# B-R-P/NMSLIB-ZIG

Hardware: AMD Instinct MI355X
Metric: queries/sec @ recall@10, 1M x 128-D L2, batch=1024; HBM GB/s vs peak (higher is better)
Workload: dtype f16+f32

## Files before the change

nmslib_zig_amd/csrc/engine.cpp:

```cpp
#include "engine.hpp"

#include <algorithm>
#include <chrono>
#include <cmath>
#include <cstring>
#include <fstream>
#include <set>
#include <sstream>
#include <thread>

namespace gfxknn {

using clk = std::chrono::steady_clock;

void hip_check(hipError_t e, const char* what) {
    if (e == hipSuccess) return;
    std::string msg = std::string(what) + ": " + hipGetErrorString(e);
    (void)hipGetLastError();
    throw EngineError(e == hipErrorOutOfMemory ? Err::OutOfMemory : Err::Runtime, msg);
}

ParamSet::ParamSet(const std::vector<std::string>& desc) {
    std::set<std::string> seen;
    for (const std::string& d : desc) {
// ... 142 lines not shown
    if (data_type != 0 && data_type != 2)
        throw EngineError(Err::SpaceIncompatible, "only dense float and dense uint8 data are served by the GPU engine");
    if ((sp == SP_L2SQR_SIFT) != (data_type == 2))
        throw EngineError(Err::SpaceIncompatible, "data type does not match space '" + space + "'");
    thread_pool_size = std::thread::hardware_concurrency();
}

Engine::~Engine() {
    for (auto& pr : prof_events_) {
        (void)hipEventDestroy(pr.first);
        (void)hipEventDestroy(pr.second);
    }
    for (hipEvent_t e : shard_events_) (void)hipEventDestroy(e);
    if (shard_ready_) (void)hipEventDestroy(shard_ready_);
    if (pinned_) (void)hipHostFree(pinned_);
    if (stream_) (void)hipStreamDestroy(stream_);
}

void Engine::prof_begin(hipStream_t s) {
    if (!prof_ || prof_events_.size() >= 65536) return;
    hipEvent_t a, b;
    hip_check(hipEventCreate(&a), "hipEventCreate");
    hip_check(hipEventCreate(&b), "hipEventCreate");
    prof_events_.emplace_back(a, b);
    hip_check(hipEventRecord(a, s), "hipEventRecord");
}
void Engine::prof_end(hipStream_t s) {
    if (!prof_ || prof_events_.empty()) return;
    hip_check(hipEventRecord(prof_events_.back().second, s), "hipEventRecord");
}
void Engine::collect_profile(double* total_ms, uint64_t* launches) {
// ... 871 lines not shown
        if (method_ == Method::Brute) knn_brute(qs, m, k, d_ids + q0 * k, d_dists + q0 * k, cnt, stream);
        else knn_hnsw(qs, m, k, d_ids + q0 * k, d_dists + q0 * k, cnt, stream);
    }
}

void Engine::fast_tile_counts(size_t* tiles, size_t* precise, size_t* fallback) {
    *tiles = *precise = *fallback = 0;
    if (!shards_.empty()) {
        shards_[0]->fast_tile_counts(tiles, precise, fallback);
        return;
    }
    if ((last_path != 1 && last_path != 3) || !fast_flags_ || fast_nqt_ <= 0) return;
    std::vector<int> h((size_t)fast_nqt_ * 2, 0);
    hip_check(hipSetDevice(device_), "hipSetDevice");
    hip_check(hipStreamSynchronize(last_stream_ ? last_stream_ : stream_), "stats");
    hip_check(hipMemcpy(h.data(), fast_flags_, (size_t)fast_nqt_ * (fast_has_precise_ ? 2 : 1) * sizeof(int), hipMemcpyDeviceToHost),
              "stats flags");
    *tiles = (size_t)fast_nqt_;
    for (int i = 0; i < fast_nqt_; ++i) {
        *fallback += h[i] != 0;
        if (fast_has_precise_) *precise += h[(size_t)fast_nqt_ + i] != 0;
    }
}

size_t Engine::hnsw_redone() {
    if (!shards_.empty()) return shards_[0]->hnsw_redone();
    if (last_path != 4 || !hnsw_fix_valid_) return 0;
    int32_t v = 0;
    hip_check(hipSetDevice(device_), "hipSetDevice");
    hip_check(hipStreamSynchronize(last_stream_ ? last_stream_ : stream_), "stats");
// ... 73 lines not shown
                ws_qaux_.ensure((size_t)f.qpad * 16);
                ws_qaug_.ensure((size_t)f.qpad * f.dp * 4);
                hip_check(launch_query_aux_cosc(ws_qpad_.as<float>(), ws_qsel_.as<float>(), f.qpad, ldb, dim_eff, mu_norm_,
                                                ws_qaux_.as<float>(), stream),
                          "query aux");
                hip_check(launch_query_aug_cosc(ws_qsel_.as<float>(), ws_qaux_.as<float>(), (int)nq, f.qpad, ldb, dim_eff,
                                                cosc_lambda_, ws_qaug_.as<float>(), f.dp, stream),
                          "augmented queries");
                qsel = ws_qaug_.as<float>();
            }
            ws_cand_.ensure(bf_cand_elems(f.fallback) * 8);
            ws_cnt_.ensure(bf_cnt_elems(f.fallback) * 4);
            ws_f32_q_.ensure((size_t)f.qpad * f.dp * 2 * 3);
            ws_u8_cand_.ensure(bf_f32_top8_elems(f) * 4);
            ws_u8_thr_.ensure(bf_f32_thr_bytes(f));
            ws_flags_.ensure((size_t)f.fallback.nqt * 4 + 64);
            ws_u8_list_.ensure(bf_f32_list_elems(f) * 4);
            ws_u8_listcnt_.ensure(bf_f32_listcnt_elems(f) * 4);
            float* thr = ws_u8_thr_.as<float>();
            int* tile_fail = reinterpret_cast<int*>(thr + 2 * (size_t)f.qpad);
            char* qh = ws_f32_q_.as<char>();
            char* ql = qh + (size_t)f.qpad * f.dp * 2;
            BfF16Side h16{d_f16_hi_.ptr(), d_auxp16_.as<float>(), ql + (size_t)f.qpad * f.dp * 2, f16_scale_, bres16_, f16_scale_q_};
            hipEvent_t eb = nullptr, ee = nullptr;
            if (prof_ && prof_events_.size() < 65536) {
                hip_check(hipEventCreate(&eb), "hipEventCreate");
                hip_check(hipEventCreate(&ee), "hipEventCreate");
                prof_events_.emplace_back(eb, ee);
            }
            hip_check(launch_bf_f32_fast(f, space_, (int)d_n_, dim_eff, ldb, (int)nq, (int)k, d_rows_.as<float>(),
                                         centred_ ? d_rows_sel_.as<float>() : d_rows_.as<float>(), d_aux_.as<float>(),
                                         d_bf_hi_.ptr(), d_bf_lo_.ptr(), d_auxp_.as<float>(), f.cosc ? bmax_c_ : bmax_,
                                         f.cosc ? bres_c_ : bres_, ws_qpad_.as<float>(), qsel, qh, ql,
                                         ws_u8_cand_.as<float>(), ws_cand_.as<unsigned long long>(), ws_cnt_.as<int>(), thr,
                                         ws_u8_list_.as<uint32_t>(), ws_u8_listcnt_.as<int>(), tile_fail, ws_flags_.as<int>(),
                                         d_ids_.as<int32_t>(), d_ids, d_dists, d_cnt, eb, ee, stream,
                                         centred_ ? nullptr : static_cast<const float*>(d_queries), centred_ ? nullptr : ws_qpad_.as<float>(),
                                         f.cosc ? ws_qaux_.as<float>() : nullptr, f.cosc ? ws_qsel_.as<float>() : nullptr, f.dp, h16),
                      "bf_f32_fast");
            last_path = 1;
            fast_flags_ = tile_fail;
            fast_nqt_ = f.nqt;
            fast_has_precise_ = true;
            return;
        }
    }
    last_path = is_u8() ? 2 : 0;
    BfPlan p = bf_make_plan((int)d_n_, dim_eff, (int)nq, (int)k, is_u8());
    if (d_n_ == 0) p.ldb = is_u8() ? 128 : f32_row_stride(dim_eff);
    const int elem = is_u8() ? 1 : 4;
    ws_qpad_.ensure((size_t)p.qpad * p.ldb * elem);
// ... 180 lines not shown
    return pinned_;
}

Engine::ResultBlock Engine::result_block(size_t nq, size_t k) {
    ws_ids_.ensure(2 * nq * k * 4 + nq * 4);
    int32_t* d_ids = ws_ids_.as<int32_t>();
    return {d_ids, reinterpret_cast<float*>(d_ids + nq * k), d_ids + 2 * nq * k};
}

void Engine::fetch_results(size_t nq, size_t k, const char* what, const int32_t** ids, const float** dists,
                           const int32_t** cnt) {
    const size_t rbytes = nq * k * 4;
    char* hp = static_cast<char*>(pinned_);
    hip_check(hipMemcpyAsync(hp, ws_ids_.ptr(), 2 * rbytes + nq * 4, hipMemcpyDeviceToHost, stream_), "results D2H");
    hip_check(hipStreamSynchronize(stream_), what);
    *ids = reinterpret_cast<const int32_t*>(hp);
    *dists = reinterpret_cast<const float*>(hp + rbytes);
    *cnt = reinterpret_cast<const int32_t*>(hp + 2 * rbytes);
}

void Engine::scan_slices(size_t nq, size_t k, int tq, const ResultBlock& out, const ScanLaunch& launch) {
    const int n = (int)d_n_;
    const size_t max_split_keys = (size_t)1 << 25;
    for (size_t q0 = 0; q0 < nq;) {
        int m = (int)std::min<size_t>(32768, nq - q0);
        ScanPlan p = scan_make_plan(n, m, (int)k, tq);
        while (m > 1 && (size_t)p.nsplit * m * k > max_split_keys) {
            m = std::max(1, m / 2);
            p = scan_make_plan(n, m, (int)k, tq);
        }
// ... 415 lines not shown
```

nmslib_zig_amd/csrc/engine.hpp:

```cpp
#pragma once
#include <hip/hip_runtime_api.h>

#include <cstdint>
#include <functional>
#include <map>
#include <memory>
#include <mutex>
#include <stdexcept>
#include <string>
#include <utility>
#include <vector>

#include "kernels/kernels.hpp"

namespace gfxknn {

enum class Err : int {
    InvalidArgument = 2,
    OutOfMemory = 3,
    SpaceIncompatible = 5,
    QueryTooLarge = 6,
    IndexBuildFailed = 8,
    QueryExecutionFailed = 9,
    DataIO = 10,
// ... 170 lines not shown
    const uint8_t* rows_u8() const { return parent_ ? parent_->rows_u8_.data() + view_lo_ * 128 : rows_u8_.data(); }
    int resolve_shards() const;
    void finalize_sharded(int nshards);
    void knn_sharded(const void* d_queries, size_t nq, size_t elem_count, size_t k, int32_t* d_ids, float* d_dists,
                     int32_t* d_cnt, hipStream_t stream);
    std::vector<std::unique_ptr<Engine>> shards_;
    std::vector<hipEvent_t> shard_events_;
    hipEvent_t shard_ready_ = nullptr;
    const Engine* parent_ = nullptr;
    size_t view_lo_ = 0, view_n_ = 0;
    int forced_device_ = -1;
    int gpu_shards_ = -1;
    DevBuf ws_sh_ids_, ws_sh_d_, ws_bigk_, ws_bigk_tmp_;
    void* pinned(size_t bytes);
    void* pinned_ = nullptr;
    size_t pinned_bytes_ = 0;
    void check_device();
    struct ResultBlock {
        int32_t* ids;
        float* dists;
        int32_t* cnt;
    };
    ResultBlock result_block(size_t nq, size_t k);
    void fetch_results(size_t nq, size_t k, const char* what, const int32_t** ids, const float** dists,
                       const int32_t** cnt);
    using ScanLaunch = std::function<void(const ScanPlan& p, size_t q0, float* split_d, int32_t* split_pos)>;
    void scan_slices(size_t nq, size_t k, int tq, const ResultBlock& out, const ScanLaunch& launch);
    using RangeLaunch = std::function<void(float* filter, float* report)>;
    size_t range_select(bool two_dists, float r, size_t capacity, int32_t* ids, float* dists, const RangeLaunch& launch);
    float read_float(const float* d_out, const char* what);
// ... 95 lines not shown
```

nmslib_zig_amd/csrc/kernels/bf_kernels.hip:

```cpp
#include <cstdio>
#include <type_traits>
#include <vector>
#include <cstdlib>

#include "common_dev.hpp"
#include "kernels.hpp"

namespace gfxknn {

enum BfMode : int { BF_L2 = 0, BF_DOT = 1, BF_COS = 2, BF_L1 = 3, BF_LINF = 4, BF_COSC = 5, BF_L2D = 6 };

struct BfArgs {
    const float* base;
    const float* aux;
    const float* qaux;
    int aux_stride;
    const float* queries;
    u64* cand;
    int* cand_cnt;
    uint32_t* gthr;
    uint32_t* gq;
    int xj, xm;
    int n, ldb, nqt, nsplit, rows_per_split, kprime, cap;
    int kcs;
// ... 152 lines not shown
    uint32_t o[8];
#pragma unroll
    for (int i = 0; i < 8; ++i) o[i] = __shfl_xor(tm[i], 32, 64);
#pragma unroll
    for (int i = 0; i < 8; ++i) ins(o[i]);
    uint32_t t = tm[0];
#pragma unroll
    for (int i = 1; i < 8; ++i) t = (i == xm - 1) ? tm[i] : t;
    return t;
}

__device__ long long g_bf_clk[2];
__device__ long long g_bf_trace[2048][3];

template <int MODE, bool FULL, bool ONE>
__global__ __launch_bounds__(256, 2) void bf_select_f32_kernel(BfArgs a) {
    extern __shared__ __attribute__((aligned(16))) char smem[];
    const int tid = threadIdx.x, lane = tid & 63, wave = tid >> 6;
    const long long clk_c0 = __builtin_readcyclecounter(), clk_r0 = wall_clock64();
    const int h = lane >> 5, l31 = lane & 31;

    const int b = blockIdx.x;
    const int xcd = b & 7, rest = b >> 3;
    const int qt = rest % a.nqt;
    const int split = (rest / a.nqt) * 8 + xcd;
    if (split >= a.nsplit) return;
    if (a.tile_fail && a.tile_fail[qt / a.fail_group] == 0) return;

    constexpr bool kDirect = (MODE == BF_L1 || MODE == BF_LINF || MODE == BF_L2D);
    constexpr bool kDelay = !kDirect;
    constexpr bool kCosC = (MODE == BF_COSC);
    constexpr int kAuxN = kCosC ? 3 : 1;
    constexpr bool kAux = (MODE == BF_L2 || MODE == BF_COS || kCosC);

    const int kcs = FULL ? BF_KC : a.kcs;
    const int lds_stride = kcs + 4;
    float* tile = reinterpret_cast<float*>(smem);
// ... 365 lines not shown
            if (a.xj > 0 && !(a.dbg & 512)) {
                if ((stage & (stage + 1)) == 0 || (stage & 31) == 31) exchange_counted();
            } else if ((stage & xmask) == xmask) {
                exchange_thr();
            }
        }
        if (!(a.dbg & 8)) __syncthreads();
    }
    if (kDelay && nstages > 0 && !skip_epi) {
        check_block(accY, 1, nstages - 1);
        if (a.xj > 0 && !(a.dbg & (256 | 512))) exchange_counted();
        if (!(a.dbg & 16)) finish_stage(true);
    }
    if (h == 0) a.cand_cnt[(size_t)qidx * a.nsplit + split] = mycnt;
    if ((a.dbg & 1024) && tid == 0) {
        if (blockIdx.x == 0) {
            g_bf_clk[0] = __builtin_readcyclecounter() - clk_c0;
            g_bf_clk[1] = wall_clock64() - clk_r0;
        }
        if (blockIdx.x < 2048) {
            g_bf_trace[blockIdx.x][0] = clk_r0;
            g_bf_trace[blockIdx.x][1] = wall_clock64();
            g_bf_trace[blockIdx.x][2] = __builtin_amdgcn_s_getreg((4 << 0) | (0 << 6) | (31 << 11));
        }
    }
}

struct BfArgsU8 {
    const uint8_t* base_i8;
    const int32_t* aux;
    const uint8_t* queries;
    u64* cand;
    int* cand_cnt;
    uint32_t* gq;
    int xj, xm;
    int n, nqt, nsplit, rows_per_split, kprime, cap;
    int dbg;
    int tile_stride;
    const int* tile_fail;
    int fail_group;
// ... 1730 lines not shown
    const int* cand_cnt;
    const int32_t* ext_ids;
    int32_t* out_ids;
    float* out_dists;
    int32_t* out_cnt;
    int space, dim, ldb, k, nsplit, cap, kprime, p2max;
    const int* tile_fail;
    int fail_queries;
    int* verify_flags;
    int verify_queries;
    const float* queries_sel;
    float bmax;
    float eps_rel;
};

__global__ __launch_bounds__(256) void bf_rerank_kernel(RerankArgs a) {
    extern __shared__ __attribute__((aligned(16))) char smem[];
    u64* keys = reinterpret_cast<u64*>(smem);
    int* offs = reinterpret_cast<int*>(keys + a.p2max);
    const int q = blockIdx.x, tid = threadIdx.x, lane = tid & 63, wave = tid >> 6;
    if (a.tile_fail && a.tile_fail[q / a.fail_queries] == 0) return;

    if (tid == 0) {
        int o = 0;
        for (int s = 0; s < a.nsplit; ++s) {
            offs[s] = o;
            int c = a.cand_cnt[(size_t)q * a.nsplit + s];
            o += c < a.kprime ? c : a.kprime;
        }
        offs[a.nsplit] = o;
    }
    __syncthreads();
    const int total = offs[a.nsplit];
    __shared__ uint32_t s_kth;
    const bool verify = a.verify_flags != nullptr && a.space == SP_L2 && total >= a.kprime;
// ... 76 lines not shown
        if (tid < 64) {
            const float* qs = a.queries_sel + (size_t)q * a.ldb;
            float ss = 0.f;
            for (int d = tid; d < a.dim; d += 64) ss = fmaf(qs[d], qs[d], ss);
            ss = wave_sum(ss);
            if (tid == 0) s_qn2v = ss;
        }
        __syncthreads();
        if (tid == 0) {
            const float qn2 = s_qn2v, qn = sqrtf(qn2);
            const float kth = ord_f32(s_kth);
            const float dk = ord_f32((uint32_t)(keys[found - 1] >> 32));
            const float e = a.eps_rel * (qn * a.bmax + 0.5f * a.bmax * a.bmax);
            const float floor_d2 = qn2 - 2.0f * kth - 2.0f * e - 2e-6f * (qn2 + fabsf(kth));
            if (!(dk * dk <= floor_d2)) atomicOr(&a.verify_flags[q / a.verify_queries], 1);
        }
    }
}

__global__ void row_aux_f32_kernel(const float* base, int n, int ldb, int dim, int space, float* aux) {
    const int lane = threadIdx.x & 63;
    const int row = blockIdx.x * (blockDim.x >> 6) + (threadIdx.x >> 6);
    if (row >= n) return;
    const float* p = base + (size_t)row * ldb;
    float s = 0.f;
    for (int d = lane; d < dim; d += 64) s = fmaf(p[d], p[d], s);
    s = wave_sum(s);
    if (lane == 0) {
        float v = 0.f;
        if (space == SP_L2) v = -0.5f * s;
// ... 523 lines not shown
                            const int* cand_cnt, const int32_t* ext_ids, int32_t* out_ids,
                            float* out_dists, int32_t* out_cnt, hipStream_t s) {
    return launch_bf_rerank_ex(p, space, dim, k, base, queries_padded, cand, cand_cnt, ext_ids, out_ids, out_dists,
                               out_cnt, nullptr, 1, s);
}

hipError_t launch_bf_rerank_ex(const BfPlan& p, int space, int dim, int k, const void* base,
                               const void* queries_padded, const unsigned long long* cand,
                               const int* cand_cnt, const int32_t* ext_ids, int32_t* out_ids,
                               float* out_dists, int32_t* out_cnt, const int* tile_fail, int fail_queries,
                               hipStream_t s) {
    return launch_bf_rerank_verify(p, space, dim, k, base, queries_padded, cand, cand_cnt, ext_ids, out_ids, out_dists,
                                   out_cnt, tile_fail, fail_queries, nullptr, nullptr, 0.f, s);
}

hipError_t launch_bf_rerank_verify(const BfPlan& p, int space, int dim, int k, const void* base,
                                   const void* queries_padded, const unsigned long long* cand,
                                   const int* cand_cnt, const int32_t* ext_ids, int32_t* out_ids,
                                   float* out_dists, int32_t* out_cnt, const int* tile_fail, int fail_queries,
                                   int* verify_flags, const float* queries_sel, float bmax, hipStream_t s) {
    RerankArgs a{};
    a.verify_flags = verify_flags;
    a.verify_queries = BF_TQ;
    a.queries_sel = queries_sel;
    a.bmax = bmax;
    a.eps_rel = 1.5f * (float)(dim + 2) * 5.9604645e-8f;
    a.tile_fail = tile_fail;
    a.fail_queries = fail_queries;
    a.base = base;
    a.queries = queries_padded;
    a.cand = cand;
    a.cand_cnt = cand_cnt;
    a.ext_ids = ext_ids;
    a.out_ids = out_ids;
    a.out_dists = out_dists;
    a.out_cnt = out_cnt;
    a.space = space;
    a.dim = dim;
    a.ldb = p.ldb;
    a.k = k;
    a.nsplit = p.nsplit;
    a.cap = p.cap;
    a.kprime = p.kprime;
    a.p2max = p.p2max;
    hipError_t e = hipFuncSetAttribute(reinterpret_cast<const void*>(bf_rerank_kernel),
                                       hipFuncAttributeMaxDynamicSharedMemorySize, (int)p.lds_rerank);
    if (e != hipSuccess) return e;
    hipLaunchKernelGGL(bf_rerank_kernel, dim3(p.nq), dim3(256), p.lds_rerank, s, a);
    return hipGetLastError();
}

hipError_t launch_bf_adaptive_f32(const BfPlan& p, int space, int dim, int k, const float* base_orig, const float* sel_rows,
                                  const float* aux, const float* queries_orig, const float* queries_sel,
                                  const float* qaux_cosc, float bmax, unsigned long long* cand, int* cand_cnt, int* flags,
                                  const int32_t* ext_ids, int32_t* out_ids, float* out_dists, int32_t* out_cnt,
                                  const int* gate, int gate_tiles, hipStream_t s, bool cleared) {
    hipError_t e = launch_bf_select_f32_ex(p, space, sel_rows, aux, queries_sel, qaux_cosc, cand, cand_cnt, gate, gate_tiles, s,
                                           cleared);
    if (e != hipSuccess) return e;
    const bool verify = space == SP_L2 && flags != nullptr && bmax > 0.f;
    if (!verify)
        return launch_bf_rerank_ex(p, space, dim, k, base_orig, queries_orig, cand, cand_cnt, ext_ids, out_ids, out_dists,
                                   out_cnt, gate, gate_tiles * BF_TQ, s);
    if (!cleared) {
        e = hipMemsetAsync(flags, 0, (size_t)p.nqt * 4, s);
        if (e != hipSuccess) return e;
    }
    e = launch_bf_rerank_verify(p, space, dim, k, base_orig, queries_orig, cand, cand_cnt, ext_ids, out_ids, out_dists,
                                out_cnt, gate, gate_tiles * BF_TQ, flags, queries_sel, bmax, s);
    if (e != hipSuccess) return e;
    e = launch_bf_select_direct_f32_ex(p, SP_L2, base_orig, queries_orig, cand, cand_cnt, flags, 1, s, cleared);
    if (e != hipSuccess) return e;
    return launch_bf_rerank_ex(p, space, dim, k, base_orig, queries_orig, cand, cand_cnt, ext_ids, out_ids, out_dists,
                               out_cnt, flags, BF_TQ, s);
}

BfU8Fast bf_u8_fast_plan(int n, int nq, int k) {
    BfU8Fast f{};
    f.use = (n >= 65536 && nq >= 512 && k <= 256);
    if (const char* e = getenv("NMSLIB_GPU_U8_FAST")) f.use = f.use && atoi(e) != 0;
    if (!f.use) return f;
    f.qg = nq >= 2048 ? 4 : 2;
    const int tq = BF_TQ * f.qg;
    f.qpad = (nq + tq - 1) / tq * tq;
    f.nqt = f.qpad / tq;
    f.stride = 8;
    if (const char* e = getenv("NMSLIB_GPU_U8_STRIDE")) f.stride = atoi(e) > 0 ? atoi(e) : 8;
    const double kf = (double)k / f.stride;
    f.r = (int)(1.6 * kf + 3.0 * sqrt(kf) + 3.0 + 0.999);
// ... 253 lines not shown
    const char* w8e = getenv("NMSLIB_GPU_BF16_W8");
    const int w8 = w8e ? atoi(w8e) : 7;
    if (sample) return (w8 & 4) ? launch_scan_bf16_one<MODE, true, 1, 8>(a, grid, lds, s) : launch_scan_bf16_one<MODE, true, 2, 4>(a, grid, lds, s);
    if (terms == 1) {
        if (qg == 2) return (w8 & 1) ? launch_scan_bf16_one<MODE, false, 2, 8>(a, grid, lds, s) : launch_scan_bf16_one<MODE, false, 4, 4>(a, grid, lds, s);
        return (w8 & 2) ? launch_scan_bf16_one<MODE, false, 1, 8>(a, grid, lds, s) : launch_scan_bf16_one<MODE, false, 2, 4>(a, grid, lds, s);
    }
    if (qg == 2) return launch_scan_f32_one<MODE, false, 4>(a, grid, lds, s);
    return launch_scan_f32_one<MODE, false, 2>(a, grid, lds, s);
}

hipError_t launch_bf_f32_fast(const BfF32Fast& f, int space, int n, int dim, int ldb, int nq, int k, const float* base_orig,
                              const float* sel_rows, const float* aux, const void* base_hi, const void* base_lo,
                              const float* auxp, float bmax, float bres, const float* queries_orig, const float* queries_sel,
                              void* q_hi, void* q_lo, float* top8, unsigned long long* cand_fb, int* cnt_fb, float* thr,
                              uint32_t* list, int* list_cnt, int* tile_fail, int* flags_fb, const int32_t* ext_ids,
                              int32_t* out_ids, float* out_dists, int32_t* out_cnt, hipEvent_t scan_begin,
                              hipEvent_t scan_end, hipStream_t s, const float* queries_raw, float* queries_pad_out,
                              const float* qaux_cosc, const float* queries_centred, int sel_ld, const BfF16Side& h16) {
    const int sdim = f.cosc ? f.sel_dim : dim, sld = f.cosc ? sel_ld : ldb;
    float* thr1 = thr + f.qpad;
    int* precise = tile_fail + f.nqt;
    hipError_t e;
    {
        const BfPlan& fb = f.fallback;
        uint32_t* gthr = reinterpret_cast<uint32_t*>(cnt_fb + (size_t)fb.qpad * fb.nsplit);
        const size_t gwords = 2 * ((size_t)fb.qpad + (size_t)fb.qpad * fb.nsplit);
        size_t work = (size_t)f.qpad * f.dp > gwords ? (size_t)f.qpad * f.dp : gwords;
        size_t grid = (work + 255) / 256;
        if (grid > 2048) grid = 2048;
        hipLaunchKernelGGL(bf_f32_prep_kernel, dim3((unsigned)grid), dim3(256), 0, s, queries_raw, nq, sdim, queries_sel, f.qpad,
                           sld, queries_pad_out, f.kch > 1 ? nullptr : static_cast<__bf16*>(q_hi),
                           f.kch > 1 ? nullptr : static_cast<__bf16*>(q_lo),
                           tile_fail, 2 * f.nqt, flags_fb, fb.nqt, gthr, gwords, f.dp, static_cast<_Float16*>(h16.q_h16), h16.scale_q);
        e = hipGetLastError();
        if (e != hipSuccess) return e;
    }
    auto scan = [&](const BfScanF32Args& sa, bool sample, int terms, int grid) -> hipError_t {
        const size_t lds = terms == 1 ? f.lds_scan1 : f.lds_scan;
        if (f.mode == 0) return launch_scan_f32_mode<SC_L2>(sa, sample, terms, f.qg, grid, lds, s, f.kch);
        if (f.mode == 1) return launch_scan_f32_mode<SC_DOT>(sa, sample, terms, f.qg, grid, lds, s, f.kch);
        return launch_scan_f32_mode<SC_COS>(sa, sample, terms, f.qg, grid, lds, s, f.kch);
    };
    BfScanF32Args a{};
    a.base_hi = static_cast<const __bf16*>(base_hi);
    a.base_lo = static_cast<const __bf16*>(base_lo);
    a.auxp = auxp;
    a.q_hi = static_cast<const __bf16*>(q_hi);
    a.q_lo = static_cast<const __bf16*>(q_lo);
// ... 122 lines not shown
            const size_t nl = (size_t)f.nsplit * 2;
            for (size_t i = 0; i < cnt.size(); ++i) {
                rows += cnt[i];
                int have = 0;
                for (int j = 0; j < f.caph && have < cnt[i]; ++j) {
                    const uint32_t e = lst[((i / nl) * f.caph + j) * nl + i % nl];
                    lx = (lx ^ e) * 1099511628211ull;
                    have += __builtin_popcount(e & 0xffffu);
                }
            }
            fprintf(stderr, "[f32fast] top8 %016llx thr %016llx thr1 %016llx flags %016llx cnt %016llx list %016llx rows %lld\n",
                    sum(top8, (size_t)f.qpad * f.s_nsplit * 2 * 8 * 4), sum(thr, (size_t)f.qpad * 4), sum(thr1, (size_t)f.qpad * 4),
                    sum(tile_fail, (size_t)f.nqt * 8), sum(list_cnt, cnt.size() * 4), lx, rows);
        }
    }
    return launch_bf_adaptive_f32(f.fallback, space, dim, k, base_orig, sel_rows, aux, queries_orig,
                                  f.cosc ? queries_centred : queries_sel, f.cosc ? qaux_cosc : nullptr, bmax,
                                  cand_fb, cnt_fb, flags_fb, ext_ids, out_ids, out_dists, out_cnt, tile_fail, f.tq / 128, s,
                                  true);
}

hipError_t launch_row_aux_f32(const float* base, int n, int ldb, int dim, int space, float* aux,
                              hipStream_t s) {
    if (n == 0) return hipSuccess;
    hipLaunchKernelGGL(row_aux_f32_kernel, dim3((n + 3) / 4), dim3(256), 0, s, base, n, ldb, dim, space, aux);
    return hipGetLastError();
}
hipError_t launch_prepare_u8(const uint8_t* base, int n, uint8_t* rows_i8, int32_t* aux, int32_t* auxh, hipStream_t s) {
    const int n_pad = bf_u8_rows_padded(n);
    hipLaunchKernelGGL(prepare_u8_kernel, dim3((n_pad + 3) / 4), dim3(256), 0, s, base, n, n_pad, rows_i8, aux, auxh);
    return hipGetLastError();
}
hipError_t launch_pad_rows(const void* src, int rows, int dim, void* dst, int rows_pad, int ld,
                           int elem_bytes, hipStream_t s) {
// ... 87 lines not shown
```

nmslib_zig_amd/csrc/kernels/kernels.hpp:

```cpp
#pragma once
#include <hip/hip_runtime_api.h>
#include <stddef.h>
#include <stdint.h>

namespace gfxknn {

enum SpaceCode : int {
    SP_L2 = 0,
    SP_L1 = 1,
    SP_LINF = 2,
    SP_COSINE = 3,
    SP_ANGULAR = 4,
    SP_NEGDOT = 5,
    SP_L2SQR_SIFT = 6,
    SP_L2SQR = 7,
    SP_NORMCOS = 8,
    SP_QNORM_NEGDOT = 9,
    SP_LEVEN = 10,
    SP_BIT_HAMMING = 11,
};

constexpr int BF_TQ = 128;
constexpr int BF_BN = 64;
constexpr int BF_KC = 128;
// ... 92 lines not shown
inline size_t bf_f32_top8_elems(const BfF32Fast& f) { return (size_t)f.qpad * f.s_nsplit * 2 * 8; }
inline int bf_f32_rows_padded(int n) { return (n + BF_BN - 1) / BF_BN * BF_BN + BF_BN; }
hipError_t launch_row_maxnorm(const float* rows, int n, int ld, int dim, bool relative_residual, float* out, hipStream_t s,
                              float scale16 = 0.f);
hipError_t launch_split_bf16(const float* src, int rows, int rows_pad, int ld, int dim, void* hi, void* lo,
                             const float* aux, float aux_pad, float* auxp, hipStream_t s, int dp = 128, void* h16 = nullptr,
                             float scale = 1.f, float* auxp16 = nullptr, float aux16_mul = 1.f);
struct BfF16Side {
    const void* base_h16;
    const float* auxp16;
    void* q_h16;
    float scale;
    float bres16;
    float scale_q;
};
hipError_t launch_bf_f32_fast(const BfF32Fast& f, int space, int n, int dim, int ldb, int nq, int k, const float* base_orig,
                              const float* sel_rows, const float* aux, const void* base_hi, const void* base_lo,
                              const float* auxp, float bmax, float bres, const float* queries_orig, const float* queries_sel,
                              void* q_hi, void* q_lo, float* top8, unsigned long long* cand_fb, int* cnt_fb, float* thr,
                              uint32_t* list, int* list_cnt, int* tile_fail, int* flags_fb, const int32_t* ext_ids, int32_t* out_ids,
                              float* out_dists, int32_t* out_cnt, hipEvent_t scan_begin, hipEvent_t scan_end,
                              hipStream_t s, const float* queries_raw = nullptr, float* queries_pad_out = nullptr,
                              const float* qaux_cosc = nullptr, const float* queries_centred = nullptr, int sel_ld = 0,
                              const BfF16Side& h16 = BfF16Side{});
hipError_t launch_row_aug_cosc(const float* orig, const float* centred, int n, int ldb, int dim, double mu_norm, float lambda,
                               float* out, int ldo, int* zero_rows, hipStream_t s);
hipError_t launch_query_aug_cosc(const float* centred, const float* qaux, int nq, int qpad, int ldb, int dim, float lambda,
                                 float* out, int ldo, hipStream_t s);

hipError_t launch_bf_adaptive_f32(const BfPlan& p, int space, int dim, int k, const float* base_orig, const float* sel_rows,
                                  const float* aux, const float* queries_orig, const float* queries_sel,
                                  const float* qaux_cosc, float bmax, unsigned long long* cand, int* cand_cnt, int* flags,
                                  const int32_t* ext_ids, int32_t* out_ids, float* out_dists, int32_t* out_cnt,
                                  const int* gate, int gate_tiles, hipStream_t s, bool cleared = false);
hipError_t launch_bf_rerank_verify(const BfPlan& p, int space, int dim, int k, const void* base,
                                   const void* queries_padded, const unsigned long long* cand,
// ... 220 lines not shown
```

Before: 2.940 million.

## Fuse brute-force fallback stages into one persistent work-queue tail kernel

Replaces the multi-launch adaptive fallback (select, rerank, verify select, verify rerank) with a single persistent kernel. Workgroups draw tickets from an atomic queue and wait on per-tile completion counters, so dependent stages can overlap across tiles instead of being serialized by kernel boundaries. The whole kernel also exits early when no tile is gated into the fallback. In exchange it adds spin-waits with a timeout that sets an abort flag and a host-mapped error word the host checks after synchronizing, and it makes correctness depend on forward progress of co-resident workgroups.

```diff
diff --git a/nmslib_zig_amd/csrc/engine.cpp b/nmslib_zig_amd/csrc/engine.cpp
--- a/nmslib_zig_amd/csrc/engine.cpp
+++ b/nmslib_zig_amd/csrc/engine.cpp
@@ -180,7 +180,25 @@
     for (hipEvent_t e : shard_events_) (void)hipEventDestroy(e);
     if (shard_ready_) (void)hipEventDestroy(shard_ready_);
     if (pinned_) (void)hipHostFree(pinned_);
+    if (tail_err_) (void)hipHostFree(tail_err_);
     if (stream_) (void)hipStreamDestroy(stream_);
+}
+
+int* Engine::tail_err_word() {
+    if (!tail_err_) {
+        hip_check(hipHostMalloc(reinterpret_cast<void**>(&tail_err_), sizeof(int), hipHostMallocPortable | hipHostMallocMapped),
+                  "hipHostMalloc");
+        *tail_err_ = 0;
+    }
+    return tail_err_;
+}
+
+void Engine::check_tail_error() {
+    for (auto& c : shards_) c->check_tail_error();
+    if (tail_err_ && *static_cast<volatile int*>(tail_err_) != 0) {
+        *tail_err_ = 0;
+        throw EngineError(Err::QueryExecutionFailed, "brute-force fallback: a stage of the tail kernel was not completed in time");
+    }
 }
 
 void Engine::prof_begin(hipStream_t s) {
@@ -1082,6 +1100,7 @@
     std::vector<int> h((size_t)fast_nqt_ * 2, 0);
     hip_check(hipSetDevice(device_), "hipSetDevice");
     hip_check(hipStreamSynchronize(last_stream_ ? last_stream_ : stream_), "stats");
+    check_tail_error();
     hip_check(hipMemcpy(h.data(), fast_flags_, (size_t)fast_nqt_ * (fast_has_precise_ ? 2 : 1) * sizeof(int), hipMemcpyDeviceToHost),
               "stats flags");
     *tiles = (size_t)fast_nqt_;
@@ -1185,7 +1204,7 @@
             ws_f32_q_.ensure((size_t)f.qpad * f.dp * 2 * 3);
             ws_u8_cand_.ensure(bf_f32_top8_elems(f) * 4);
             ws_u8_thr_.ensure(bf_f32_thr_bytes(f));
-            ws_flags_.ensure((size_t)f.fallback.nqt * 4 + 64);
+            ws_flags_.ensure(bf_f32_flags_elems(f) * 4 + 64);
             ws_u8_list_.ensure(bf_f32_list_elems(f) * 4);
             ws_u8_listcnt_.ensure(bf_f32_listcnt_elems(f) * 4);
             float* thr = ws_u8_thr_.as<float>();
@@ -1205,7 +1224,7 @@
                                          f.cosc ? bres_c_ : bres_, ws_qpad_.as<float>(), qsel, qh, ql,
                                          ws_u8_cand_.as<float>(), ws_cand_.as<unsigned long long>(), ws_cnt_.as<int>(), thr,
                                          ws_u8_list_.as<uint32_t>(), ws_u8_listcnt_.as<int>(), tile_fail, ws_flags_.as<int>(),
-                                         d_ids_.as<int32_t>(), d_ids, d_dists, d_cnt, eb, ee, stream,
+                                         tail_err_word(), d_ids_.as<int32_t>(), d_ids, d_dists, d_cnt, eb, ee, stream,
                                          centred_ ? nullptr : static_cast<const float*>(d_queries), centred_ ? nullptr : ws_qpad_.as<float>(),
                                          f.cosc ? ws_qaux_.as<float>() : nullptr, f.cosc ? ws_qsel_.as<float>() : nullptr, f.dp, h16),
                       "bf_f32_fast");
@@ -1416,6 +1435,7 @@
     char* hp = static_cast<char*>(pinned_);
     hip_check(hipMemcpyAsync(hp, ws_ids_.ptr(), 2 * rbytes + nq * 4, hipMemcpyDeviceToHost, stream_), "results D2H");
     hip_check(hipStreamSynchronize(stream_), what);
+    check_tail_error();
     *ids = reinterpret_cast<const int32_t*>(hp);
     *dists = reinterpret_cast<const float*>(hp + rbytes);
     *cnt = reinterpret_cast<const int32_t*>(hp + 2 * rbytes);
diff --git a/nmslib_zig_amd/csrc/engine.hpp b/nmslib_zig_amd/csrc/engine.hpp
--- a/nmslib_zig_amd/csrc/engine.hpp
+++ b/nmslib_zig_amd/csrc/engine.hpp
@@ -208,6 +208,9 @@
     DevBuf ws_sh_ids_, ws_sh_d_, ws_bigk_, ws_bigk_tmp_;
     void* pinned(size_t bytes);
     void* pinned_ = nullptr;
+    int* tail_err_ = nullptr;
+    int* tail_err_word();
+    void check_tail_error();
     size_t pinned_bytes_ = 0;
     void check_device();
     struct ResultBlock {
diff --git a/nmslib_zig_amd/csrc/kernels/bf_kernels.hip b/nmslib_zig_amd/csrc/kernels/bf_kernels.hip
--- a/nmslib_zig_amd/csrc/kernels/bf_kernels.hip
+++ b/nmslib_zig_amd/csrc/kernels/bf_kernels.hip
@@ -3,6 +3,7 @@
 #include <vector>
 #include <cstdlib>
 
+#include "bf_tail_queue.hpp"
 #include "common_dev.hpp"
 #include "kernels.hpp"
 
@@ -190,13 +191,11 @@
 __device__ long long g_bf_trace[2048][3];
 
 template <int MODE, bool FULL, bool ONE>
-__global__ __launch_bounds__(256, 2) void bf_select_f32_kernel(BfArgs a) {
-    extern __shared__ __attribute__((aligned(16))) char smem[];
+__device__ __forceinline__ void bf_select_f32_body(const BfArgs& a, const int b, char* smem) {
     const int tid = threadIdx.x, lane = tid & 63, wave = tid >> 6;
     const long long clk_c0 = __builtin_readcyclecounter(), clk_r0 = wall_clock64();
     const int h = lane >> 5, l31 = lane & 31;
 
-    const int b = blockIdx.x;
     const int xcd = b & 7, rest = b >> 3;
     const int qt = rest % a.nqt;
     const int split = (rest / a.nqt) * 8 + xcd;
@@ -592,16 +591,22 @@
     }
     if (h == 0) a.cand_cnt[(size_t)qidx * a.nsplit + split] = mycnt;
     if ((a.dbg & 1024) && tid == 0) {
-        if (blockIdx.x == 0) {
+        if (b == 0) {
             g_bf_clk[0] = __builtin_readcyclecounter() - clk_c0;
             g_bf_clk[1] = wall_clock64() - clk_r0;
         }
-        if (blockIdx.x < 2048) {
-            g_bf_trace[blockIdx.x][0] = clk_r0;
-            g_bf_trace[blockIdx.x][1] = wall_clock64();
-            g_bf_trace[blockIdx.x][2] = __builtin_amdgcn_s_getreg((4 << 0) | (0 << 6) | (31 << 11));
-        }
-    }
+        if (b < 2048) {
+            g_bf_trace[b][0] = clk_r0;
+            g_bf_trace[b][1] = wall_clock64();
+            g_bf_trace[b][2] = __builtin_amdgcn_s_getreg((4 << 0) | (0 << 6) | (31 << 11));
+        }
+    }
+}
+
+template <int MODE, bool FULL, bool ONE>
+__global__ __launch_bounds__(256, 2) void bf_select_f32_kernel(BfArgs a) {
+    extern __shared__ __attribute__((aligned(16))) char smem[];
+    bf_select_f32_body<MODE, FULL, ONE>(a, blockIdx.x, smem);
 }
 
 struct BfArgsU8 {
@@ -2362,11 +2367,10 @@
     float eps_rel;
 };
 
-__global__ __launch_bounds__(256) void bf_rerank_kernel(RerankArgs a) {
-    extern __shared__ __attribute__((aligned(16))) char smem[];
+__device__ __forceinline__ void bf_rerank_body(const RerankArgs& a, const int q, char* smem) {
     u64* keys = reinterpret_cast<u64*>(smem);
     int* offs = reinterpret_cast<int*>(keys + a.p2max);
-    const int q = blockIdx.x, tid = threadIdx.x, lane = tid & 63, wave = tid >> 6;
+    const int tid = threadIdx.x, lane = tid & 63, wave = tid >> 6;
     if (a.tile_fail && a.tile_fail[q / a.fail_queries] == 0) return;
 
     if (tid == 0) {
@@ -2473,6 +2477,121 @@
             const float e = a.eps_rel * (qn * a.bmax + 0.5f * a.bmax * a.bmax);
             const float floor_d2 = qn2 - 2.0f * kth - 2.0f * e - 2e-6f * (qn2 + fabsf(kth));
             if (!(dk * dk <= floor_d2)) atomicOr(&a.verify_flags[q / a.verify_queries], 1);
+        }
+    }
+}
+
+__global__ __launch_bounds__(256) void bf_rerank_kernel(RerankArgs a) {
+    extern __shared__ __attribute__((aligned(16))) char smem[];
+    bf_rerank_body(a, blockIdx.x, smem);
+}
+
+struct BfTailArgs {
+    BfArgs sel;
+    BfArgs sel_d;
+    RerankArgs rr;
+    BfTailQueue q;
+    const int* gate;
+    int gate_tiles, ngate;
+    int* words;
+    int* err;
+    long long wait_ticks;
+};
+
+typedef const BfTailArgs __attribute__((address_space(4)))* BfTailArgsPtr;
+__device__ __forceinline__ BfTailArgsPtr bf_tail_args() {
+    BfTailArgsPtr p = (BfTailArgsPtr)__builtin_amdgcn_kernarg_segment_ptr();
+    asm volatile("" : "+s"(p));
+    return p;
+}
+template <class T>
+__device__ __forceinline__ T bf_tail_ld(const T __attribute__((address_space(4)))* src) {
+    T v;
+    __builtin_memcpy(&v, src, sizeof(T));
+    return v;
+}
+
+__device__ __forceinline__ int bf_tail_wait(const BfTailQueue& q, int* words, int* err, long long wait_ticks, int stage, int tile) {
+    const int want = bf_tail_producers(q, stage, tile);
+    int* word = words + bf_tail_done_word(q, stage, tile);
+    const long long t0 = wall_clock64();
+    for (;;) {
+        if (__hip_atomic_load(word, __ATOMIC_ACQUIRE, __HIP_MEMORY_SCOPE_AGENT) >= want) return 1;
+        if (__hip_atomic_load(words + BF_TAIL_ABORT, __ATOMIC_RELAXED, __HIP_MEMORY_SCOPE_AGENT) != 0) return -1;
+        if (wall_clock64() - t0 > wait_ticks) {
+            __hip_atomic_store(words + BF_TAIL_ABORT, 1, __ATOMIC_RELAXED, __HIP_MEMORY_SCOPE_AGENT);
+            __hip_atomic_fetch_or(err, 1, __ATOMIC_RELAXED, __HIP_MEMORY_SCOPE_SYSTEM);
+            return -1;
+        }
+        __builtin_amdgcn_s_sleep(32);
+    }
+}
+
+template <int MODE, bool FULL, bool ONE>
+__global__ __launch_bounds__(256, 2) void bf_tail_f32_kernel(BfTailArgs) {
+    extern __shared__ __attribute__((aligned(16))) char smem[];
+    __shared__ int s_ticket, s_go;
+    const int tid = threadIdx.x;
+    {
+        BfTailArgsPtr p = bf_tail_args();
+        const int* gate = p->gate;
+        const int ngate = p->ngate;
+        int any = 0;
+        for (int i = tid; i < ngate; i += blockDim.x) any |= gate[i];
+        if (!__syncthreads_or(any)) return;
+    }
+    for (;;) {
+        __syncthreads();
+        BfTailArgsPtr p = bf_tail_args();
+        const BfTailQueue q = bf_tail_ld(&p->q);
+        int* words = p->words;
+        const int total = bf_tail_total(q);
+        if (tid == 0) {
+            const int t = atomicAdd(words + BF_TAIL_HEAD, 1);
+            int go = 0;
+            if (t < total) {
+                const BfTailItem it = bf_tail_decode(q, t);
+                int* err = p->err;
+                const long long wait_ticks = p->wait_ticks;
+                go = p->gate[it.tile / p->gate_tiles] != 0;
+                if (go && it.stage > 0) go = bf_tail_wait(q, words, err, wait_ticks, it.stage < 3 ? it.stage - 1 : 1, it.tile);
+                if (go > 0 && it.stage >= 2) {
+                    go = __hip_atomic_load(p->rr.verify_flags + it.tile, __ATOMIC_RELAXED, __HIP_MEMORY_SCOPE_AGENT) != 0;
+                    if (go && it.stage == 3) go = bf_tail_wait(q, words, err, wait_ticks, 2, it.tile);
+                }
+            }
+            s_ticket = t;
+            s_go = go;
+        }
+        __syncthreads();
+        const int t = s_ticket, go = s_go;
+        if (t >= total) break;
+        if (go == 0) continue;
+        const BfTailItem it = bf_tail_decode(q, t);
+        if (go < 0) {
+            int32_t* out_cnt = p->rr.out_cnt;
+            if (!bf_tail_is_select(it.stage) && tid == 0 && out_cnt) out_cnt[it.index] = 0;
+            continue;
+        }
+        if (it.stage > 0) __builtin_amdgcn_fence(__ATOMIC_ACQUIRE, "agent");
+        if (it.stage == 0) {
+            const BfArgs sa = bf_tail_ld(&bf_tail_args()->sel);
+            bf_select_f32_body<MODE, FULL, ONE>(sa, it.index, smem);
+        } else if (it.stage == 2) {
+            if constexpr (MODE == BF_L2) {
+                const BfArgs sa = bf_tail_ld(&bf_tail_args()->sel_d);
+                bf_select_f32_body<BF_L2D, false, false>(sa, it.index, smem);
+            }
+        } else {
+            RerankArgs r = bf_tail_ld(&bf_tail_args()->rr);
+            if (it.stage == 3) r.verify_flags = nullptr;
+            bf_rerank_body(r, it.index, smem);
+        }
+        __threadfence();
+        __syncthreads();
+        if (tid == 0) {
+            __threadfence();
+            atomicAdd(bf_tail_args()->words + bf_tail_done_word(q, it.stage, it.tile), 1);
         }
     }
 }
@@ -3026,11 +3145,10 @@
                                    out_cnt, tile_fail, fail_queries, nullptr, nullptr, 0.f, s);
 }
 
-hipError_t launch_bf_rerank_verify(const BfPlan& p, int space, int dim, int k, const void* base,
-                                   const void* queries_padded, const unsigned long long* cand,
-                                   const int* cand_cnt, const int32_t* ext_ids, int32_t* out_ids,
-                                   float* out_dists, int32_t* out_cnt, const int* tile_fail, int fail_queries,
-                                   int* verify_flags, const float* queries_sel, float bmax, hipStream_t s) {
+static RerankArgs make_rerank_args(const BfPlan& p, int space, int dim, int k, const void* base, const void* queries_padded,
+                                   const unsigned long long* cand, const int* cand_cnt, const int32_t* ext_ids,
+                                   int32_t* out_ids, float* out_dists, int32_t* out_cnt, const int* tile_fail,
+                                   int fail_queries, int* verify_flags, const float* queries_sel, float bmax) {
     RerankArgs a{};
     a.verify_flags = verify_flags;
     a.verify_queries = BF_TQ;
@@ -3055,6 +3173,16 @@
     a.cap = p.cap;
     a.kprime = p.kprime;
     a.p2max = p.p2max;
+    return a;
+}
+
+hipError_t launch_bf_rerank_verify(const BfPlan& p, int space, int dim, int k, const void* base,
+                                   const void* queries_padded, const unsigned long long* cand,
+                                   const int* cand_cnt, const int32_t* ext_ids, int32_t* out_ids,
+                                   float* out_dists, int32_t* out_cnt, const int* tile_fail, int fail_queries,
+                                   int* verify_flags, const float* queries_sel, float bmax, hipStream_t s) {
+    const RerankArgs a = make_rerank_args(p, space, dim, k, base, queries_padded, cand, cand_cnt, ext_ids, out_ids, out_dists,
+                                          out_cnt, tile_fail, fail_queries, verify_flags, queries_sel, bmax);
     hipError_t e = hipFuncSetAttribute(reinterpret_cast<const void*>(bf_rerank_kernel),
                                        hipFuncAttributeMaxDynamicSharedMemorySize, (int)p.lds_rerank);
     if (e != hipSuccess) return e;
@@ -3085,6 +3213,95 @@
     if (e != hipSuccess) return e;
     return launch_bf_rerank_ex(p, space, dim, k, base_orig, queries_orig, cand, cand_cnt, ext_ids, out_ids, out_dists,
                                out_cnt, flags, BF_TQ, s);
+}
+
+template <int MODE, bool FULL, bool ONE>
+static hipError_t launch_tail_kern(const BfTailArgs& a, int grid, size_t lds, hipStream_t s) {
+    auto kern = bf_tail_f32_kernel<MODE, FULL, ONE>;
+    hipError_t e = hipFuncSetAttribute(reinterpret_cast<const void*>(kern), hipFuncAttributeMaxDynamicSharedMemorySize, (int)lds);
+    if (e != hipSuccess) return e;
+    hipLaunchKernelGGL(kern, dim3(grid), dim3(256), lds, s, a);
+    return hipGetLastError();
+}
+
+template <int MODE>
+static hipError_t launch_tail_mode(const BfPlan& p, const BfTailArgs& a, int grid, size_t lds, hipStream_t s) {
+#ifdef BF_FAST_COMPILE
+    if (MODE == BF_L2 && p.ldb == BF_KC) return launch_tail_kern<BF_L2, true, true>(a, grid, lds, s);
+    return hipErrorInvalidValue;
+#else
+    if (p.ldb == BF_KC) return launch_tail_kern<MODE, true, true>(a, grid, lds, s);
+    if (p.ldb % BF_KC == 0) return launch_tail_kern<MODE, true, false>(a, grid, lds, s);
+    return launch_tail_kern<MODE, false, false>(a, grid, lds, s);
+#endif
+}
+
+static hipError_t launch_bf_tail_f32(const BfPlan& p, int space, int dim, int k, const float* base_orig, const float* sel_rows,
+                                     const float* aux, const float* queries_orig, const float* queries_sel,
+                                     const float* qaux_cosc, float bmax, unsigned long long* cand, int* cand_cnt, int* flags,
+                                     const int32_t* ext_ids, int32_t* out_ids, float* out_dists, int32_t* out_cnt,
+                                     const int* gate, int gate_tiles, int* err, hipStream_t s) {
+    if (!gate || !flags || !err || gate_tiles < 1) return hipErrorInvalidValue;
+    const bool verify = space == SP_L2 && bmax > 0.f;
+    uint32_t* gthr = reinterpret_cast<uint32_t*>(cand_cnt + (size_t)p.qpad * p.nsplit);
+    const size_t gwords = (size_t)p.qpad + (size_t)p.qpad * p.nsplit;
+    BfTailArgs a{};
+    a.sel = make_args(p, sel_rows, aux, queries_sel, cand, cand_cnt, gthr);
+    a.sel_d = make_args(p, base_orig, nullptr, queries_orig, cand, cand_cnt, gthr + gwords);
+    a.rr = make_rerank_args(p, space, dim, k, base_orig, queries_orig, cand, cand_cnt, ext_ids, out_ids, out_dists, out_cnt,
+                            nullptr, 1, verify ? flags : nullptr, verify ? queries_sel : nullptr, verify ? bmax : 0.f);
+    a.q.nqt = p.nqt;
+    a.q.nsplit = p.nsplit;
+    a.q.nq = p.nq;
+    a.q.nstages = verify ? 4 : 2;
+    a.gate = gate;
+    a.gate_tiles = gate_tiles;
+    a.ngate = (p.nqt + gate_tiles - 1) / gate_tiles;
+    a.words = flags + p.nqt;
+    a.err = err;
+    a.wait_ticks = 20ll * 100000000ll;
+    static int cus[64] = {0};
+    int dev = 0;
+    hipError_t e = hipGetDevice(&dev);
+    if (e != hipSuccess) return e;
+    if (dev < 0 || dev >= 64) return hipErrorInvalidValue;
+    if (cus[dev] == 0) {
+        e = hipDeviceGetAttribute(&cus[dev], hipDeviceAttributeMultiprocessorCount, dev);
+        if (e != hipSuccess) return e;
+    }
+    const int total = bf_tail_total(a.q);
+    int grid = 2 * cus[dev];
+    if (grid > total) grid = total;
+    if (grid < 1) grid = 1;
+    const size_t lds = p.lds_select > p.lds_rerank ? p.lds_select : p.lds_rerank;
+    switch (space) {
+        case SP_L2: e = launch_tail_mode<BF_L2>(p, a, grid, lds, s); break;
+        case SP_NEGDOT: e = launch_tail_mode<BF_DOT>(p, a, grid, lds, s); break;
+        case SP_COSINE:
+        case SP_ANGULAR:
+            if (qaux_cosc) {
+                a.sel.qaux = qaux_cosc;
+                a.sel.aux_stride = p.n;
+                e = launch_tail_mode<BF_COSC>(p, a, grid, lds, s);
+            } else {
+                e = launch_tail_mode<BF_COS>(p, a, grid, lds, s);
+            }
+            break;
+        default: return hipErrorInvalidValue;
+    }
+    const char* te = getenv("NMSLIB_GPU_TAIL_TRACE");
+    const bool trace = te && atoi(te);
+    if (trace && e == hipSuccess) {
+        std::vector<int> w((size_t)bf_tail_words(p.nqt));
+        (void)hipStreamSynchronize(s);
+        (void)hipMemcpy(w.data(), a.words, w.size() * 4, hipMemcpyDeviceToHost);
+        long long done[4] = {0, 0, 0, 0};
+        for (int st = 0; st < 4; ++st)
+            for (int t = 0; t < p.nqt; ++t) done[st] += w[(size_t)bf_tail_done_word(a.q, st, t)];
+        fprintf(stderr, "[bf tail] workgroups %d tickets %d drawn %d abort %d items done: stage0 %lld stage1 %lld stage2 %lld stage3 %lld\n",
+                grid, total, w[BF_TAIL_HEAD], w[BF_TAIL_ABORT], done[0], done[1], done[2], done[3]);
+    }
+    return e;
 }
 
 BfU8Fast bf_u8_fast_plan(int n, int nq, int k) {
@@ -3368,8 +3585,8 @@
                               const float* sel_rows, const float* aux, const void* base_hi, const void* base_lo,
                               const float* auxp, float bmax, float bres, const float* queries_orig, const float* queries_sel,
                               void* q_hi, void* q_lo, float* top8, unsigned long long* cand_fb, int* cnt_fb, float* thr,
-                              uint32_t* list, int* list_cnt, int* tile_fail, int* flags_fb, const int32_t* ext_ids,
-                              int32_t* out_ids, float* out_dists, int32_t* out_cnt, hipEvent_t scan_begin,
+                              uint32_t* list, int* list_cnt, int* tile_fail, int* flags_fb, int* tail_err,
+                              const int32_t* ext_ids, int32_t* out_ids, float* out_dists, int32_t* out_cnt, hipEvent_t scan_begin,
                               hipEvent_t scan_end, hipStream_t s, const float* queries_raw, float* queries_pad_out,
                               const float* qaux_cosc, const float* queries_centred, int sel_ld, const BfF16Side& h16) {
     const int sdim = f.cosc ? f.sel_dim : dim, sld = f.cosc ? sel_ld : ldb;
@@ -3386,7 +3603,7 @@
         hipLaunchKernelGGL(bf_f32_prep_kernel, dim3((unsigned)grid), dim3(256), 0, s, queries_raw, nq, sdim, queries_sel, f.qpad,
                            sld, queries_pad_out, f.kch > 1 ? nullptr : static_cast<__bf16*>(q_hi),
                            f.kch > 1 ? nullptr : static_cast<__bf16*>(q_lo),
-                           tile_fail, 2 * f.nqt, flags_fb, fb.nqt, gthr, gwords, f.dp, static_cast<_Float16*>(h16.q_h16), h16.scale_q);
+                           tile_fail, 2 * f.nqt, flags_fb, fb.nqt + bf_tail_words(fb.nqt), gthr, gwords, f.dp, static_cast<_Float16*>(h16.q_h16), h16.scale_q);
         e = hipGetLastError();
         if (e != hipSuccess) return e;
     }
@@ -3539,10 +3756,9 @@
                     sum(tile_fail, (size_t)f.nqt * 8), sum(list_cnt, cnt.size() * 4), lx, rows);
         }
     }
-    return launch_bf_adaptive_f32(f.fallback, space, dim, k, base_orig, sel_rows, aux, queries_orig,
-                                  f.cosc ? queries_centred : queries_sel, f.cosc ? qaux_cosc : nullptr, bmax,
-                                  cand_fb, cnt_fb, flags_fb, ext_ids, out_ids, out_dists, out_cnt, tile_fail, f.tq / 128, s,
-                                  true);
+    return launch_bf_tail_f32(f.fallback, space, dim, k, base_orig, sel_rows, aux, queries_orig,
+                              f.cosc ? queries_centred : queries_sel, f.cosc ? qaux_cosc : nullptr, bmax,
+                              cand_fb, cnt_fb, flags_fb, ext_ids, out_ids, out_dists, out_cnt, tile_fail, f.tq / 128, tail_err, s);
 }
 
 hipError_t launch_row_aux_f32(const float* base, int n, int ldb, int dim, int space, float* aux,
diff --git a/nmslib_zig_amd/csrc/kernels/bf_tail_queue.hpp b/nmslib_zig_amd/csrc/kernels/bf_tail_queue.hpp
--- /dev/null
+++ b/nmslib_zig_amd/csrc/kernels/bf_tail_queue.hpp
@@ -0,0 +1,67 @@
+#pragma once
+
+#if defined(__HIPCC__)
+#define BF_TAIL_HD __host__ __device__ inline
+#else
+#define BF_TAIL_HD inline
+#endif
+
+namespace gfxknn {
+
+constexpr int BF_TAIL_TQ = 128;
+
+struct BfTailQueue {
+    int nqt;
+    int nsplit;
+    int nq;
+    int nstages;
+};
+
+struct BfTailItem {
+    int stage;
+    int index;
+    int tile;
+    int part;
+};
+
+BF_TAIL_HD bool bf_tail_is_select(int stage) { return (stage & 1) == 0; }
+BF_TAIL_HD int bf_tail_stage_items(const BfTailQueue& q, int stage) { return bf_tail_is_select(stage) ? q.nqt * q.nsplit : q.nq; }
+BF_TAIL_HD int bf_tail_first_ticket(const BfTailQueue& q, int stage) {
+    int t = 0;
+    for (int s = 0; s < stage; ++s) t += bf_tail_stage_items(q, s);
+    return t;
+}
+BF_TAIL_HD int bf_tail_total(const BfTailQueue& q) { return bf_tail_first_ticket(q, q.nstages); }
+
+BF_TAIL_HD int bf_tail_select_tile(const BfTailQueue& q, int index) { return (index >> 3) % q.nqt; }
+BF_TAIL_HD int bf_tail_select_split(const BfTailQueue& q, int index) { return ((index >> 3) / q.nqt) * 8 + (index & 7); }
+
+BF_TAIL_HD BfTailItem bf_tail_decode(const BfTailQueue& q, int ticket) {
+    BfTailItem it;
+    it.stage = 0;
+    it.index = ticket;
+    while (it.stage + 1 < q.nstages && it.index >= bf_tail_stage_items(q, it.stage)) {
+        it.index -= bf_tail_stage_items(q, it.stage);
+        ++it.stage;
+    }
+    if (bf_tail_is_select(it.stage)) {
+        it.tile = bf_tail_select_tile(q, it.index);
+        it.part = bf_tail_select_split(q, it.index);
+    } else {
+        it.tile = it.index / BF_TAIL_TQ;
+        it.part = it.index % BF_TAIL_TQ;
+    }
+    return it;
+}
+
+BF_TAIL_HD int bf_tail_producers(const BfTailQueue& q, int stage, int tile) {
+    if (bf_tail_is_select(stage)) return q.nsplit;
+    const int left = q.nq - tile * BF_TAIL_TQ;
+    return left < 0 ? 0 : (left < BF_TAIL_TQ ? left : BF_TAIL_TQ);
+}
+
+constexpr int BF_TAIL_HEAD = 0, BF_TAIL_ABORT = 1, BF_TAIL_DONE = 2;
+BF_TAIL_HD int bf_tail_done_word(const BfTailQueue& q, int stage, int tile) { return BF_TAIL_DONE + stage * q.nqt + tile; }
+BF_TAIL_HD int bf_tail_words(int nqt) { return BF_TAIL_DONE + 4 * nqt; }
+
+}
diff --git a/nmslib_zig_amd/csrc/kernels/kernels.hpp b/nmslib_zig_amd/csrc/kernels/kernels.hpp
--- a/nmslib_zig_amd/csrc/kernels/kernels.hpp
+++ b/nmslib_zig_amd/csrc/kernels/kernels.hpp
@@ -2,6 +2,8 @@
 #include <hip/hip_runtime_api.h>
 #include <stddef.h>
 #include <stdint.h>
+
+#include "bf_tail_queue.hpp"
 
 namespace gfxknn {
 
@@ -130,12 +132,13 @@
     float bres16;
     float scale_q;
 };
+inline size_t bf_f32_flags_elems(const BfF32Fast& f) { return (size_t)f.fallback.nqt + (size_t)bf_tail_words(f.fallback.nqt); }
 hipError_t launch_bf_f32_fast(const BfF32Fast& f, int space, int n, int dim, int ldb, int nq, int k, const float* base_orig,
                               const float* sel_rows, const float* aux, const void* base_hi, const void* base_lo,
                               const float* auxp, float bmax, float bres, const float* queries_orig, const float* queries_sel,
                               void* q_hi, void* q_lo, float* top8, unsigned long long* cand_fb, int* cnt_fb, float* thr,
-                              uint32_t* list, int* list_cnt, int* tile_fail, int* flags_fb, const int32_t* ext_ids, int32_t* out_ids,
-                              float* out_dists, int32_t* out_cnt, hipEvent_t scan_begin, hipEvent_t scan_end,
+                              uint32_t* list, int* list_cnt, int* tile_fail, int* flags_fb, int* tail_err, const int32_t* ext_ids,
+                              int32_t* out_ids, float* out_dists, int32_t* out_cnt, hipEvent_t scan_begin, hipEvent_t scan_end,
                               hipStream_t s, const float* queries_raw = nullptr, float* queries_pad_out = nullptr,
                               const float* qaux_cosc = nullptr, const float* queries_centred = nullptr, int sel_ld = 0,
                               const BfF16Side& h16 = BfF16Side{});
```

Result: no change. 3.005 million (median of 4 runs) (+2.2%).
